# PeterFWS/Structure-PLP-SLAM

Measured on NVIDIA H100. Metric: frames_per_sec_extract_match_poseopt, higher is better.
Workload: dtype u8/f64

## Files before the change

### structure-plp-slam_b200/csrc/orb.cu

```cuda
#include "common.cuh"
#include <cuda.h>
#include <stdlib.h>
#include "brief_pattern.inc"
#include "quadtree_kernels.cuh"

namespace plp {

namespace {

constexpr int kMaxLevels = 16;
constexpr int kHalfPatch = 15;
constexpr int kCellSize = 64;
constexpr int kOverlap = 6;

struct LevelInfo {
    int w, h, pitch;
    size_t offset;
    size_t blur_offset;
    int cells_x, cells_y;
    int cell_base;
    int num_cells;
    int budget;
    int slot_base;
    int slot_cap;
    float scale_factor;
    float size;
};

struct CellDesc {
    short level, i, j, pad;
    short min_x, min_y, max_x, max_y;
};

struct BlurTile {
    short level, x0, y0, pad;
};

struct OrbDev {
    int num_levels, rows, cols;
    int num_cells;
    int total_slots;
    int out_cap;
    int ini_thr, min_thr;
    LevelInfo lv[kMaxLevels];
    int u_max[16];
    const uint8_t *img0;
    size_t img0_step, img0_frame_stride;
    const uint8_t *mask;
    size_t mask_step;
    uint8_t *pyr;
    size_t pyr_frame_bytes;
    uint8_t *blur;
    size_t blur_frame_bytes;
    const BlurTile *blur_tiles;
    int num_blur_tiles;
    const CellDesc *cells;
    uint32_t *cell_buf;
    int *cell_cnt;
    LevelKp *lvl_kp;
    int *lvl_cnt;
    uint8_t *qt_scratch;
    size_t qt_scratch_per_job;
    int *status;
};

__device__ __forceinline__ const uint8_t *level_ptr(const OrbDev &P, int b, int l) {
    return l == 0 ? P.img0 + (size_t)b * P.img0_frame_stride : P.pyr + (size_t)b * P.pyr_frame_bytes + P.lv[l].offset;
}
__device__ __forceinline__ int level_pitch(const OrbDev &P, int l) { return l == 0 ? (int)P.img0_step : P.lv[l].pitch; }

constexpr int kBtW = 64, kBtH = 32;
constexpr int kBoxW = 96, kBoxH = kBtH + 6, kBoxX = 16;
static_assert(kBoxW >= kBoxX + kBtW + 3 && kBoxW % 16 == 0 && kBoxX % 16 == 0 && kBtW % 16 == 0,
              "TMA box: 16-byte aligned start and extent covering the 3-pixel halo");
static_assert(kBoxH % 2 == 0 && kBtH % 2 == 0, "the blur passes work on pairs of rows");
constexpr int kBoxStage = (kBoxH * kBoxW + 127) & ~127;
constexpr int kTilePitch = kBoxW;
constexpr int kTileRows = kCellSize + kOverlap;

struct BlurMaps {
    CUtensorMap m[kMaxLevels];
};

__device__ __forceinline__ uint32_t smem_u32(const void *p) { return (uint32_t)__cvta_generic_to_shared(p); }

__device__ __forceinline__ void mbar_init(uint32_t bar) { asm volatile("mbarrier.init.shared::cta.b64 [%0], 1;" ::"r"(bar)); }

__device__ __forceinline__ bool mbar_wait(uint32_t bar, uint32_t parity) {
    uint32_t done = 0;
    for (int spin = 0; spin < (1 << 14) && !done; ++spin)
        asm volatile(
            "{\n\t.reg .pred p;\n\tmbarrier.try_wait.parity.shared::cta.b64 p, [%1], %2;\n\tselp.u32 %0, 1, 0, p;\n\t}"
            : "=r"(done)
            : "r"(bar), "r"(parity)
            : "memory");
    return done != 0;
}

__device__ __forceinline__ void mbar_expect_tx(uint32_t bar, uint32_t bytes) {
    asm volatile("mbarrier.arrive.expect_tx.shared::cta.b64 _, [%0], %1;" ::"r"(bar), "r"(bytes) : "memory");
}

__device__ __forceinline__ void tma_box_load(uint32_t dst, const CUtensorMap *tm, int x, int y, int f, uint32_t bar) {
    asm volatile(
        "cp.async.bulk.tensor.3d.shared::cluster.global.mbarrier::complete_tx::bytes [%0], [%1, {%2, %3, %4}], [%5];"
        ::"r"(dst), "l"(tm), "r"(x), "r"(y), "r"(f), "r"(bar)
        : "memory");
}

constexpr int kResizeRows = 8;
__global__ void __launch_bounds__(256) pyr_resize_kernel(OrbDev P, int l, const short4 *__restrict__ xtab,
                                                         const short4 *__restrict__ ytab) {
    const int b = blockIdx.y;
    const int dw = P.lv[l].w, dh = P.lv[l].h, dpitch = P.lv[l].pitch;
    const int quads = (dw + 3) >> 2, strips = (dh + kResizeRows - 1) / kResizeRows;
    const int q = blockIdx.x * blockDim.x + threadIdx.x;
    if (q >= quads * strips) return;
    const int strip = q / quads, x0 = (q - strip * quads) * 4;
    const uint8_t *src = level_ptr(P, b, l - 1);
    const int spitch = level_pitch(P, l - 1);
    uint8_t *dst = const_cast<uint8_t *>(level_ptr(P, b, l));
    int sx0[4], sx1[4], a0[4], a1[4];
#pragma unroll
    for (int k = 0; k < 4; ++k) {
        const short4 xt = xtab[min(x0 + k, dw - 1)];
        sx0[k] = xt.x;
        sx1[k] = xt.y;
        a0[k] = xt.z;
        a1[k] = xt.w;
    }
    const int y_end = min(dh, (strip + 1) * kResizeRows);
    for (int y = strip * kResizeRows; y < y_end; ++y) {
        const short4 yt = ytab[y];
        const uint8_t *S0 = src + (size_t)yt.x * spitch, *S1 = src + (size_t)yt.y * spitch;
        const int b0 = yt.z, b1 = yt.w;
        uint32_t packed = 0;
#pragma unroll
        for (int k = 0; k < 4; ++k) {
            const int r0 = S0[sx0[k]] * a0[k] + S0[sx1[k]] * a1[k];
            const int r1 = S1[sx0[k]] * a0[k] + S1[sx1[k]] * a1[k];
            const int v = (((b0 * (r0 >> 4)) >> 16) + ((b1 * (r1 >> 4)) >> 16) + 2) >> 2;
            packed |= (uint32_t)(v & 0xff) << (8 * k);
        }
        *reinterpret_cast<uint32_t *>(dst + (size_t)y * dpitch + x0) = packed;
    }
}

__device__ __forceinline__ uint32_t fast_m_pair(const uint8_t *pa, const uint8_t *pb) {
    const uint32_t v2 = ((uint32_t)pa[0] + 256u) | (((uint32_t)pb[0] + 256u) << 16);
    uint32_t d[16];
#define PLP_RING(k, off) d[k] = v2 - ((uint32_t)pa[off] | ((uint32_t)pb[off] << 16))
    PLP_RING(0, 3 * kTilePitch);
    PLP_RING(1, 3 * kTilePitch + 1);
    PLP_RING(2, 2 * kTilePitch + 2);
    PLP_RING(3, 1 * kTilePitch + 3);
    PLP_RING(4, 3);
    PLP_RING(5, -1 * kTilePitch + 3);
    PLP_RING(6, -2 * kTilePitch + 2);
    PLP_RING(7, -3 * kTilePitch + 1);
    PLP_RING(8, -3 * kTilePitch);
    PLP_RING(9, -3 * kTilePitch - 1);
    PLP_RING(10, -2 * kTilePitch - 2);
    PLP_RING(11, -1 * kTilePitch - 3);
    PLP_RING(12, -3);
    PLP_RING(13, 1 * kTilePitch - 3);
    PLP_RING(14, 2 * kTilePitch - 2);
    PLP_RING(15, 3 * kTilePitch - 1);
#undef PLP_RING
    uint32_t e[16], d2[16], e2[16], d4[16], e4[16];
#pragma unroll
    for (int k = 0; k < 16; ++k) e[k] = 0x02000200u - d[k];
#pragma unroll
    for (int k = 0; k < 16; ++k) {
        d2[k] = __vimin3_s16x2(d[k], d[(k + 1) & 15], d[(k + 1) & 15]);
        e2[k] = __vimin3_s16x2(e[k], e[(k + 1) & 15], e[(k + 1) & 15]);
    }
#pragma unroll
    for (int k = 0; k < 16; ++k) {
        d4[k] = __vimin3_s16x2(d2[k], d2[(k + 2) & 15], d2[(k + 2) & 15]);
        e4[k] = __vimin3_s16x2(e2[k], e2[(k + 2) & 15], e2[(k + 2) & 15]);
    }
    uint32_t best = 0u;
#pragma unroll
    for (int k = 0; k < 16; ++k) {
        const uint32_t d9 = __vimin3_s16x2(d4[k], d4[(k + 4) & 15], d[(k + 8) & 15]);
        const uint32_t e9 = __vimin3_s16x2(e4[k], e4[(k + 4) & 15], e[(k + 8) & 15]);
        best = __vimax3_s16x2(best, d9, e9);
    }
    return best;
}

__device__ __forceinline__ bool masked(const OrbDev &P, unsigned y, unsigned x, float scale) {
    return P.mask[(size_t)(int)(y * scale) * P.mask_step + (int)(x * scale)] == 0;
}


constexpr int kTileX = kPatchRadius % 16;
constexpr int kTestX = kTileX + 3;
static_assert(kCellSize % 16 == 0 && kTestX % 4 == 2, "the pretests below form their words for tested x = 2 (mod 4)");
static_assert(kTileX + kCellSize + kOverlap <= kTilePitch, "a cell row fits a tile row");
constexpr int kFastBox2Row = kTileRows - kBoxH;
static_assert(kFastBox2Row > 0 && kFastBox2Row <= kBoxH && (kFastBox2Row * kTilePitch) % 128 == 0,
              "two boxes cover the tile rows; the second lands 128-byte aligned");
constexpr int kFastStage = (kTileRows * kTilePitch + 127) & ~127;
constexpr int kCornerWords = 4;
static_assert(kCornerWords * 32 >= kTilePitch + 32, "corner bitmap row");

#define PLP_TW(y, k) T32[(y) * (kTilePitch / 4) + (k)]

__device__ __forceinline__ uint32_t compass4(const uint32_t *T32, int y, int k, uint32_t t4) {
    const uint32_t c = __funnelshift_r(PLP_TW(y, k), PLP_TW(y, k + 1), 16);
    const uint32_t up = __funnelshift_r(PLP_TW(y - 3, k), PLP_TW(y - 3, k + 1), 16);
    const uint32_t dn = __funnelshift_r(PLP_TW(y + 3, k), PLP_TW(y + 3, k + 1), 16);
    const uint32_t lf = __funnelshift_r(PLP_TW(y, k - 1), PLP_TW(y, k), 24);
    const uint32_t rt = __funnelshift_r(PLP_TW(y, k + 1), PLP_TW(y, k + 2), 8);
    const uint32_t a0 = __vcmpgtu4(__vabsdiffu4(c, dn), t4), a4 = __vcmpgtu4(__vabsdiffu4(c, rt), t4);
    const uint32_t a8 = __vcmpgtu4(__vabsdiffu4(c, up), t4), a12 = __vcmpgtu4(__vabsdiffu4(c, lf), t4);
    const uint32_t sv = (a4 | a12) & (a0 | a8);
    const uint32_t m = sv & 0x01010101u;
    return (m | (m >> 7) | (m >> 14) | (m >> 21)) & 0xfu;
}

__device__ __forceinline__ uint32_t even8_4(const uint32_t *T32, int y, int k, uint32_t k7) {
    const uint32_t c = __funnelshift_r(PLP_TW(y, k), PLP_TW(y, k + 1), 16);
    auto gt = [&](uint32_t ring) -> uint32_t {
        const uint32_t d = __vabsdiffu4(c, ring);
        return (((d & 0x7f7f7f7fu) + k7) | d) & 0x80808080u;
    };
    const uint32_t e0 = gt(__funnelshift_r(PLP_TW(y + 3, k), PLP_TW(y + 3, k + 1), 16));
    const uint32_t e2 = gt(PLP_TW(y + 2, k + 1));
// ... 554 lines not shown
                const uint32_t r[12] = {q0.x, q0.y, q0.z, q0.w, q1.x, q1.y, q1.z, q1.w, q2.x, q2.y, q2.z, q2.w};
                const int od = (cx - kHalfPatch) & 15, sh = 8 * (od & 3);
                switch (od >> 2) {
                    case 0: disc_row_sums<0>(r, sh, wu, wm, su, si); break;
                    case 1: disc_row_sums<1>(r, sh, wu, wm, su, si); break;
                    case 2: disc_row_sums<2>(r, sh, wu, wm, su, si); break;
                    default: disc_row_sums<3>(r, sh, wu, wm, su, si); break;
                }
            }
            int m10 = su, m01 = (lane - kHalfPatch) * si;
#pragma unroll
            for (int o = 16; o > 0; o >>= 1) {
                m10 += __shfl_xor_sync(0xffffffffu, m10, o);
                m01 += __shfl_xor_sync(0xffffffffu, m01, o);
            }
            const float angle = fast_atan2_deg((float)m01, (float)m10);

            const float ang_rad = (float)((double)angle * 3.14159265358979323846 / 180.0);
            const float ca = util_cos(ang_rad), sa = util_sin(ang_rad);
            const uint8_t *center = win + kWinHalf * kWinPitch + kWinHalf + ((cx - kWinHalf) & 15);
            int val = 0;
#pragma unroll
            for (int bit = 0; bit < 8; ++bit) {
                const int r1 = __float2int_rn(x1[bit] * sa + y1[bit] * ca), c1 = __float2int_rn(x1[bit] * ca - y1[bit] * sa);
                const int r2 = __float2int_rn(x2[bit] * sa + y2[bit] * ca), c2 = __float2int_rn(x2[bit] * ca - y2[bit] * sa);
                val |= (center[r1 * kWinPitch + c1] < center[r2 * kWinPitch + c2]) << bit;
            }
            desc_out[((size_t)b * P.out_cap + p0 + i) * 32 + lane] = (uint8_t)val;
            if (lane == i) my_angle = angle;
            __syncwarp();
        }
        if (lane < n) {
            plp_keypoint o;
            const float s = s_scale[ml];
            o.x = ml == 0 ? (float)mx : (float)mx * s;
            o.y = ml == 0 ? (float)my : (float)my * s;
            o.size = s_size[ml];
            o.angle = my_angle;
            o.response = (float)mresp;
            o.octave = ml;
            o.class_id = -1;
            kp_out[(size_t)b * P.out_cap + p0 + lane] = o;
        }
    }
}

}

}

using namespace plp;

constexpr auto kQtSmall = quadtree_kernel<kNodeCapSmall, kCandCapSmall, kQtThreadsSmall, kQtMinBlocksSmall>;
constexpr auto kQtLarge = quadtree_kernel<kNodeCap, kCandCapLarge, kQtThreadsLarge, kQtMinBlocksLarge>;
static_assert(kQtMaxLevels >= kMaxLevels, "the quadtree job holds every pyramid level");

static QtJob qt_job(const OrbDev &D) {
    QtJob J;
    J.num_levels = D.num_levels;
    J.num_cells = D.num_cells;
    J.total_slots = D.total_slots;
    for (int l = 0; l < D.num_levels; ++l) {
        const LevelInfo &V = D.lv[l];
        J.lv[l] = QtLevel{V.w, V.h, V.cell_base, V.num_cells, V.budget, V.slot_base, V.slot_cap};
    }
    J.cell_buf = D.cell_buf;
    J.cell_cnt = D.cell_cnt;
    J.lvl_kp = D.lvl_kp;
    J.lvl_cnt = D.lvl_cnt;
    J.scratch = D.qt_scratch;
    J.scratch_per_job = D.qt_scratch_per_job;
    J.status = D.status;
    return J;
}

struct plp_orb {
    plp_ctx *ctx = nullptr;
    plp_orb_params params;
    int rows = 0, cols = 0, max_batch = 0;
    OrbDev dev;
    std::vector<float> scale_factors, inv_scale_factors, level_sigma_sq, inv_level_sigma_sq;
    std::vector<uint32_t> num_keypts_per_level;
    std::vector<CellDesc> cells;
    short4 *d_xtab[kMaxLevels] = {nullptr};
    short4 *d_ytab[kMaxLevels] = {nullptr};
    CellDesc *d_cells = nullptr;
    uint8_t *d_pyr = nullptr;
    uint8_t *d_blur = nullptr;
    BlurTile *d_blur_tiles = nullptr;
    std::vector<BlurTile> blur_tiles;
    uint8_t *d_img = nullptr;
    uint8_t *d_mask = nullptr;
    uint32_t *d_cell_buf = nullptr;
    int *d_cell_cnt = nullptr;
    LevelKp *d_lvl_kp = nullptr;
    int *d_lvl_cnt = nullptr;
    uint8_t *d_qt_scratch = nullptr;
    int *d_status = nullptr;
    plp_keypoint *d_kp = nullptr;
    uint8_t *d_desc = nullptr;
    int32_t *d_n = nullptr;
    size_t qt_smem = 0;
    bool qt_small = false;
    BlurMaps maps;
    bool maps_ok = false;
    const uint8_t *map0_img = nullptr;
    size_t map0_step = 0;
    int map0_batch = 0;
    int last_batch = 0;
    const uint8_t *last_img0 = nullptr;
    size_t last_step = 0;
};

typedef CUresult (*EncodeTiledFn)(CUtensorMap *, CUtensorMapDataType, cuuint32_t, void *, const cuuint64_t *, const cuuint64_t *,
                                  const cuuint32_t *, const cuuint32_t *, CUtensorMapInterleave, CUtensorMapSwizzle,
                                  CUtensorMapL2promotion, CUtensorMapFloatOOBfill);
static EncodeTiledFn tensor_map_encoder() {
    static EncodeTiledFn fn = []() -> EncodeTiledFn {
        void *p = nullptr;
        cudaDriverEntryPointQueryResult q;
        if (cudaGetDriverEntryPoint("cuTensorMapEncodeTiled", &p, cudaEnableDefault, &q) != cudaSuccess ||
            q != cudaDriverEntryPointSuccess)
            return nullptr;
        return (EncodeTiledFn)p;
    }();
    return fn;
}
static bool encode_level_map(CUtensorMap *m, const uint8_t *base, int w, int h, int frames, size_t pitch, size_t frame_stride) {
    EncodeTiledFn enc = tensor_map_encoder();
    if (!enc || ((uintptr_t)base & 15) || (pitch & 15) || (frame_stride & 15) || w < 1 || h < 1 || frames < 1) return false;
    const cuuint64_t dims[3] = {(cuuint64_t)w, (cuuint64_t)h, (cuuint64_t)frames};
    const cuuint64_t strides[2] = {(cuuint64_t)pitch, (cuuint64_t)frame_stride};
    const cuuint32_t box[3] = {(cuuint32_t)kBoxW, (cuuint32_t)kBoxH, 1u}, estr[3] = {1u, 1u, 1u};
    return enc(m, CU_TENSOR_MAP_DATA_TYPE_UINT8, 3, (void *)base, dims, strides, box, estr, CU_TENSOR_MAP_INTERLEAVE_NONE,
               CU_TENSOR_MAP_SWIZZLE_NONE, CU_TENSOR_MAP_L2_PROMOTION_L2_128B, CU_TENSOR_MAP_FLOAT_OOB_FILL_NONE) == CUDA_SUCCESS;
}


static void build_resize_tables(int sw, int sh, int dw, int dh, std::vector<short4> &xt, std::vector<short4> &yt) {
    const double inv_scale_x = (double)dw / sw, inv_scale_y = (double)dh / sh;
    const double scale_x = 1. / inv_scale_x, scale_y = 1. / inv_scale_y;
    xt.resize(dw);
    yt.resize(dh);
    for (int dx = 0; dx < dw; ++dx) {
        float fx = (float)((dx + 0.5) * scale_x - 0.5);
        int sx = cv_floor(fx);
        fx -= sx;
        if (sx < 0) {
            fx = 0;
            sx = 0;
        }
        if (sx >= sw - 1) {
            fx = 0;
            sx = sw - 1;
        }
        short4 t;
        t.x = (short)sx;
        t.y = (short)std::min(sx + 1, sw - 1);
        t.z = (short)lrintf((1.f - fx) * 2048);
        t.w = (short)lrintf(fx * 2048);
        xt[dx] = t;
    }
    for (int dy = 0; dy < dh; ++dy) {
        float fy = (float)((dy + 0.5) * scale_y - 0.5);
        int sy = cv_floor(fy);
        fy -= sy;
        short4 t;
        t.x = (short)std::min(std::max(sy, 0), sh - 1);
        t.y = (short)std::min(std::max(sy + 1, 0), sh - 1);
        t.z = (short)lrintf((1.f - fy) * 2048);
        t.w = (short)lrintf(fy * 2048);
        yt[dy] = t;
    }
}

extern "C" {

void plp_orb_destroy(plp_orb *o) {
    if (!o) return;
    cudaSetDevice(o->ctx->device);
    cudaStreamSynchronize(o->ctx->stream);
    for (int l = 0; l < kMaxLevels; ++l) {
        if (o->d_xtab[l]) cudaFree(o->d_xtab[l]);
        if (o->d_ytab[l]) cudaFree(o->d_ytab[l]);
    }
    void *ptrs[] = {o->d_blur, o->d_blur_tiles, o->d_cells, o->d_pyr, o->d_img, o->d_mask, o->d_cell_buf, o->d_cell_cnt, o->d_lvl_kp,
                    o->d_lvl_cnt, o->d_qt_scratch, o->d_status, o->d_kp, o->d_desc, o->d_n};
    for (void *p : ptrs)
        if (p) cudaFree(p);
    delete o;
}

plp_status plp_orb_create(plp_ctx *ctx, const plp_orb_params *params, int rows, int cols, int max_batch,
                          plp_orb **out) {
    PLP_REQUIRE(ctx && params && out, "null pointer");
    *out = nullptr;
    PLP_REQUIRE(rows > 0 && cols > 0 && max_batch > 0, "image size / batch");
    PLP_REQUIRE(params->num_levels >= 1 && params->num_levels <= kMaxLevels, "num_levels in [1,16]");
    PLP_REQUIRE(params->scale_factor > 1.0f || params->num_levels == 1, "scale_factor > 1");
    PLP_REQUIRE(cols <= 2047 + 2 * kPatchRadius && rows <= 1023 + 2 * kPatchRadius,
                "image larger than 2085 x 1061 (packed candidate coordinates)");
    PLP_REQUIRE(params->ini_fast_thr < 255 && params->min_fast_thr >= 1 && params->min_fast_thr <= params->ini_fast_thr,
                "FAST thresholds: 1 <= min <= ini < 255");
    PLP_CUDA_TRY(cudaSetDevice(ctx->device));
    plp_orb *o = new plp_orb();
    o->ctx = ctx;
    o->params = *params;
    o->rows = rows;
    o->cols = cols;
    o->max_batch = max_batch;
    const unsigned L = params->num_levels;
    o->scale_factors.assign(L, 1.0f);
    o->inv_scale_factors.assign(L, 1.0f);
    o->level_sigma_sq.assign(L, 1.0f);
    o->inv_level_sigma_sq.assign(L, 1.0f);
    for (unsigned l = 1; l < L; ++l) o->scale_factors[l] = params->scale_factor * o->scale_factors[l - 1];
    for (unsigned l = 1; l < L; ++l) o->inv_scale_factors[l] = (1.0f / params->scale_factor) * o->inv_scale_factors[l - 1];
    {
        float s = 1.0f;
        for (unsigned l = 1; l < L; ++l) {
            s = params->scale_factor * s;
            o->level_sigma_sq[l] = s * s;
            o->inv_level_sigma_sq[l] = 1.0f / (s * s);
        }
    }
    o->num_keypts_per_level.resize(L);
    {
        double desired = params->max_num_keypts * (1.0 - 1.0 / params->scale_factor) /
                         (1.0 - std::pow(1.0 / params->scale_factor, static_cast<double>(L)));
        if (L == 1) desired = params->max_num_keypts;
        unsigned total = 0;
        for (unsigned l = 0; l + 1 < L; ++l) {
            o->num_keypts_per_level[l] = (unsigned)std::round(desired);
            total += o->num_keypts_per_level[l];
            desired *= 1.0 / params->scale_factor;
        }
        o->num_keypts_per_level[L - 1] = (unsigned)std::max((int)params->max_num_keypts - (int)total, 0);
    }
    OrbDev &D = o->dev;
    memset(&D, 0, sizeof(D));
    D.num_levels = (int)L;
    D.rows = rows;
    D.cols = cols;
    D.ini_thr = (int)params->ini_fast_thr;
    D.min_thr = (int)params->min_fast_thr;
    {
        const unsigned vmax = (unsigned)std::floor(kHalfPatch * std::sqrt(2.0) / 2 + 1);
        const unsigned vmin = (unsigned)std::ceil(kHalfPatch * std::sqrt(2.0) / 2);
        for (unsigned v = 0; v <= vmax; ++v)
            D.u_max[v] = (int)std::round(std::sqrt((double)kHalfPatch * kHalfPatch - (double)v * v));
        for (unsigned v = kHalfPatch, v0 = 0; vmin <= v; --v) {
            while (D.u_max[v0] == D.u_max[v0 + 1]) ++v0;
            D.u_max[v] = (int)v0;
            ++v0;
        }
    }
    int qt_max_slots = 0, qt_max_cells = 0;
    size_t pyr_bytes = 0, blur_bytes = 0;
    int slot_base = 0, cell_base = 0;
    plp_status st = PLP_OK;
    for (unsigned l = 0; l < L; ++l) {
        LevelInfo &V = D.lv[l];
        if (l == 0) {
            V.w = cols;
            V.h = rows;
        } else {
            const double scale = o->scale_factors[l];
            V.w = (int)std::round(cols * 1.0 / scale);
            V.h = (int)std::round(rows * 1.0 / scale);
// ... 5 lines not shown
        V.blur_offset = blur_bytes;
        blur_bytes += (size_t)V.pitch * V.h + 256;
        blur_bytes = (blur_bytes + 255) & ~(size_t)255;
        for (int y0 = 0; y0 < V.h; y0 += kBtH)
            for (int x0 = 0; x0 < V.w; x0 += kBtW) o->blur_tiles.push_back(BlurTile{(short)l, (short)x0, (short)y0, 0});
        V.budget = (int)o->num_keypts_per_level[l];
        V.scale_factor = o->scale_factors[l];
        V.size = (float)(unsigned)(31 * o->scale_factors[l]);
        V.slot_base = slot_base;
        {
            int g0 = 1;
            if (V.w > 2 * kPatchRadius && V.h > 2 * kPatchRadius) {
                const double ratio = (double)(V.w - 2 * kPatchRadius) / (V.h - 2 * kPatchRadius);
                g0 = ratio > 1 ? (int)std::round(ratio) : (int)std::round(1 / ratio);
            }
            V.slot_cap = 4 * std::max(V.budget, g0) + 8;
        }
        slot_base += V.slot_cap;
        V.cell_base = cell_base;
        V.num_cells = 0;
        qt_max_slots = std::max(qt_max_slots, V.slot_cap);
        if (V.slot_cap > kNodeCap) {
            set_error("orb: level %u budget %d exceeds the quadtree node capacity", l, V.budget);
            st = PLP_ERR_CAPACITY;
        }
        if (V.w > 2 * kPatchRadius && V.h > 2 * kPatchRadius && V.w >= 1 && V.h >= 1) {
            const unsigned min_bx = kPatchRadius, min_by = kPatchRadius;
            const unsigned max_bx = V.w - kPatchRadius, max_by = V.h - kPatchRadius;
            const unsigned width = max_bx - min_bx, height = max_by - min_by;
            const unsigned ncols = width / kCellSize + 1, nrows = height / kCellSize + 1;
            V.cells_x = (int)ncols;
            V.cells_y = (int)nrows;
            for (unsigned i = 0; i < nrows; ++i) {
                const unsigned min_y = min_by + i * kCellSize;
                if (max_by - kOverlap <= min_y || max_by < kOverlap) continue;
                unsigned max_y = min_y + kCellSize + kOverlap;
                if (max_by < max_y) max_y = max_by;
                for (unsigned j = 0; j < ncols; ++j) {
                    const unsigned min_x = min_bx + j * kCellSize;
                    if (max_bx - kOverlap <= min_x || max_bx < kOverlap) continue;
                    unsigned max_x = min_x + kCellSize + kOverlap;
                    if (max_bx < max_x) max_x = max_bx;
                    CellDesc c;
                    c.level = (short)l;
                    c.i = (short)i;
                    c.j = (short)j;
                    c.pad = 0;
                    c.min_x = (short)min_x;
                    c.min_y = (short)min_y;
                    c.max_x = (short)max_x;
                    c.max_y = (short)max_y;
                    o->cells.push_back(c);
                    V.num_cells++;
                }
            }
        }
        cell_base += V.num_cells;
        qt_max_cells = std::max(qt_max_cells, V.num_cells);
    }
    if (st == PLP_OK && qt_max_cells + 1 > 2 * (qt_max_slots <= kNodeCapSmall ? kNodeCapSmall : kNodeCap)) {
        set_error("orb: a pyramid level of %d FAST cells exceeds the quadtree's cell capacity", qt_max_cells);
        st = PLP_ERR_CAPACITY;
    }
    if (st != PLP_OK) {
        delete o;
        return st;
    }
    D.num_cells = cell_base;
    D.total_slots = slot_base;
    D.out_cap = slot_base;
    D.pyr_frame_bytes = pyr_bytes ? pyr_bytes : 256;
    D.blur_frame_bytes = blur_bytes ? blur_bytes : 256;
    D.num_blur_tiles = (int)o->blur_tiles.size();
    const size_t B = (size_t)max_batch;
#define ORB_ALLOC(ptr, bytes)                                              \
    do {                                                                   \
        cudaError_t e_ = cudaMalloc((void **)&(ptr), (bytes) ? (bytes) : 256); \
        if (e_ != cudaSuccess) {                                           \
            set_error("orb: cudaMalloc(%zu) failed: %s", (size_t)(bytes), cudaGetErrorString(e_)); \
            plp_orb_destroy(o);                                            \
            return PLP_ERR_CUDA;                                           \
        }                                                                  \
    } while (0)
    for (unsigned l = 1; l < L; ++l) {
        std::vector<short4> xt, yt;
        build_resize_tables(D.lv[l - 1].w, D.lv[l - 1].h, D.lv[l].w, D.lv[l].h, xt, yt);
        ORB_ALLOC(o->d_xtab[l], xt.size() * sizeof(short4));
        ORB_ALLOC(o->d_ytab[l], yt.size() * sizeof(short4));
        cudaMemcpy(o->d_xtab[l], xt.data(), xt.size() * sizeof(short4), cudaMemcpyHostToDevice);
        cudaMemcpy(o->d_ytab[l], yt.data(), yt.size() * sizeof(short4), cudaMemcpyHostToDevice);
    }
    ORB_ALLOC(o->d_cells, o->cells.size() * sizeof(CellDesc));
    if (!o->cells.empty())
        cudaMemcpy(o->d_cells, o->cells.data(), o->cells.size() * sizeof(CellDesc), cudaMemcpyHostToDevice);
    ORB_ALLOC(o->d_pyr, B * D.pyr_frame_bytes);
    ORB_ALLOC(o->d_blur, B * D.blur_frame_bytes);
    ORB_ALLOC(o->d_blur_tiles, o->blur_tiles.size() * sizeof(BlurTile));
    if (!o->blur_tiles.empty())
        cudaMemcpy(o->d_blur_tiles, o->blur_tiles.data(), o->blur_tiles.size() * sizeof(BlurTile), cudaMemcpyHostToDevice);
    ORB_ALLOC(o->d_img, B * (size_t)rows * cols);
    ORB_ALLOC(o->d_mask, (size_t)rows * cols);
    ORB_ALLOC(o->d_cell_buf, B * (size_t)D.num_cells * kCellCap * sizeof(uint32_t));
    ORB_ALLOC(o->d_cell_cnt, B * (size_t)D.num_cells * sizeof(int));
    ORB_ALLOC(o->d_lvl_kp, B * (size_t)D.total_slots * sizeof(LevelKp));
    ORB_ALLOC(o->d_lvl_cnt, B * L * sizeof(int));
    D.qt_scratch_per_job = qt_scratch_bytes_per_job();
    ORB_ALLOC(o->d_qt_scratch, B * L * D.qt_scratch_per_job);
    ORB_ALLOC(o->d_status, B * sizeof(int));
    ORB_ALLOC(o->d_kp, B * (size_t)D.out_cap * sizeof(plp_keypoint));
    ORB_ALLOC(o->d_desc, B * (size_t)D.out_cap * 32);
    ORB_ALLOC(o->d_n, B * sizeof(int32_t));
#undef ORB_ALLOC
    D.pyr = o->d_pyr;
    D.blur = o->d_blur;
    D.blur_tiles = o->d_blur_tiles;
    D.cells = o->d_cells;
    D.cell_buf = o->d_cell_buf;
    D.cell_cnt = o->d_cell_cnt;
    D.lvl_kp = o->d_lvl_kp;
    D.lvl_cnt = o->d_lvl_cnt;
    D.qt_scratch = o->d_qt_scratch;
    D.status = o->d_status;
    o->maps_ok = true;
    memset(&o->maps, 0, sizeof(o->maps));
    for (unsigned l = 1; l < L && o->maps_ok; ++l)
        o->maps_ok = encode_level_map(&o->maps.m[l], o->d_pyr + D.lv[l].offset, D.lv[l].w, D.lv[l].h, max_batch, D.lv[l].pitch,
                                      D.pyr_frame_bytes);
    o->qt_small = qt_max_slots <= kNodeCapSmall;
    plp_status so;
    if (o->qt_small) {
        o->qt_smem = qt_smem_bytes<kNodeCapSmall, kCandCapSmall, kQtThreadsSmall>();
        so = ensure_smem_optin((const void *)kQtSmall, o->qt_smem, "quadtree_kernel<small>");
    } else {
        o->qt_smem = qt_smem_bytes<kNodeCap, kCandCapLarge, kQtThreadsLarge>();
        so = ensure_smem_optin((const void *)kQtLarge, o->qt_smem, "quadtree_kernel<large>");
    }
    if (so != PLP_OK) {
        plp_orb_destroy(o);
        return so;
    }
    *out = o;
    return PLP_OK;
}

int plp_orb_capacity(const plp_orb *o) { return o ? o->dev.out_cap : 0; }

plp_status plp_orb_get_tables(const plp_orb *o, float *sf, float *isf, float *ls, float *ils, uint32_t *nk) {
    PLP_REQUIRE(o, "orb");
    for (int l = 0; l < o->dev.num_levels; ++l) {
        if (sf) sf[l] = o->scale_factors[l];
        if (isf) isf[l] = o->inv_scale_factors[l];
        if (ls) ls[l] = o->level_sigma_sq[l];
        if (ils) ils[l] = o->inv_level_sigma_sq[l];
        if (nk) nk[l] = o->num_keypts_per_level[l];
    }
    return PLP_OK;
}

static plp_status orb_run(plp_orb *o, const uint8_t *d_imgs, int batch, size_t step, const uint8_t *d_mask,
                          size_t mask_step, plp_keypoint *d_kp, uint8_t *d_desc, int32_t *d_n, int32_t *d_status) {
    plp_ctx *ctx = o->ctx;
    OrbDev D = o->dev;
    D.img0 = d_imgs;
    D.img0_step = step;
    D.img0_frame_stride = step * (size_t)o->rows;
    D.mask = d_mask;
    D.mask_step = mask_step;
    D.status = d_status ? d_status : o->d_status;
    o->last_batch = batch;
    o->last_img0 = d_imgs;
    o->last_step = step;
    PLP_CUDA_TRY(cudaMemsetAsync(D.status, 0, (size_t)batch * sizeof(int), ctx->stream));
    for (int l = 1; l < D.num_levels; ++l) {
        const int quads = ((D.lv[l].w + 3) >> 2) * ((D.lv[l].h + kResizeRows - 1) / kResizeRows);
        if (quads <= 0) continue;
        dim3 grid(div_up(quads, 256), batch);
        PLP_LAUNCH(ctx, pyr_resize_kernel, grid, 256, 0, D, l, o->d_xtab[l], o->d_ytab[l]);
    }
    bool tma = o->maps_ok;
    if (tma && (o->map0_img != d_imgs || o->map0_step != step || o->map0_batch != batch)) {
        tma = encode_level_map(&o->maps.m[0], d_imgs, D.lv[0].w, D.lv[0].h, batch, step, D.img0_frame_stride);
        o->map0_img = tma ? d_imgs : nullptr;
        o->map0_step = step;
        o->map0_batch = batch;
    }
    if (D.num_cells > 0) {
        dim3 grid(D.num_cells, batch), grid_run(div_up(D.num_cells, kFastRun), batch);
        if (tma)
            PLP_LAUNCH(ctx, fast_cells_tma_kernel, grid_run, 256, 0, o->maps, D, kFastRun);
        else
            PLP_LAUNCH(ctx, fast_cells_kernel_v2, grid, 256, 0, D);
    }
    if (D.num_blur_tiles > 0) {
        dim3 grid(D.num_blur_tiles, batch), grid_run(div_up(D.num_blur_tiles, kBlurRun), batch);
        if (tma)
            PLP_LAUNCH(ctx, blur_tiles_tma_kernel, grid_run, kBlurThreads, 0, o->maps, D, kBlurRun);
        else
            PLP_LAUNCH(ctx, blur_tiles_kernel, grid, kBlurThreads, 0, D);
    }
    {
        dim3 grid(D.num_levels, batch);
        if (ctx->timing) plp::timing_begin(ctx, o->qt_small ? "quadtree_kernel<1024>" : "quadtree_kernel<2048>");
        const QtJob J = qt_job(D);
        if (o->qt_small)
            kQtSmall<<<grid, kQtThreadsSmall, o->qt_smem, ctx->stream>>>(J);
        else
            kQtLarge<<<grid, kQtThreadsLarge, o->qt_smem, ctx->stream>>>(J);
        if (ctx->timing) plp::timing_end(ctx);
        ctx->launches++;
    }
    {
        const int kp_est = std::max(256, (int)o->params.max_num_keypts);
        dim3 grid(div_up(std::min(D.total_slots, kp_est), kDescWarps * kDescRun), batch);
        PLP_LAUNCH(ctx, describe_kernel, grid, kDescWarps * 32, 0, D, d_kp, d_desc, d_n);
    }
    PLP_CHECK_LAUNCH();
    return PLP_OK;
}

plp_status plp_orb_extract_batch_dev(plp_orb *o, const uint8_t *d_imgs, int batch, size_t step, plp_keypoint *d_kp,
                                     uint8_t *d_desc, int32_t *d_n, int32_t *d_status) {
    PLP_REQUIRE(o && d_imgs && d_kp && d_desc && d_n, "null pointer");
    PLP_REQUIRE(batch >= 1 && batch <= o->max_batch, "batch exceeds the handle's max_batch");
    PLP_REQUIRE(step >= (size_t)o->cols, "step < cols");
    PLP_CUDA_TRY(cudaSetDevice(o->ctx->device));
    return orb_run(o, d_imgs, batch, step, nullptr, 0, d_kp, d_desc, d_n, d_status);
}

static plp_status orb_extract_host(plp_orb *o, const uint8_t *imgs, int batch, size_t step, const uint8_t *mask,
                                   size_t mask_step, plp_keypoint *kp_out, uint8_t *desc_out, int32_t *n_out) {
    plp_ctx *ctx = o->ctx;
    PLP_CUDA_TRY(cudaSetDevice(ctx->device));
    const size_t rows = o->rows, cols = o->cols;
    PLP_CUDA_TRY(cudaMemcpy2DAsync(o->d_img, cols, imgs, step, cols, rows * (size_t)batch, cudaMemcpyHostToDevice,
                                   ctx->stream));
    const uint8_t *d_mask = nullptr;
    if (mask) {
        PLP_CUDA_TRY(cudaMemcpy2DAsync(o->d_mask, cols, mask, mask_step, cols, rows, cudaMemcpyHostToDevice, ctx->stream));
        d_mask = o->d_mask;
    }
    PLP_TRY(orb_run(o, o->d_img, batch, cols, d_mask, cols, o->d_kp, o->d_desc, o->d_n, nullptr));
    const size_t cap = o->dev.out_cap;
    PLP_CUDA_TRY(cudaMemcpyAsync(n_out, o->d_n, (size_t)batch * 4, cudaMemcpyDeviceToHost, ctx->stream));
    PLP_CUDA_TRY(cudaMemcpyAsync(kp_out, o->d_kp, (size_t)batch * cap * sizeof(plp_keypoint), cudaMemcpyDeviceToHost,
                                 ctx->stream));
    PLP_CUDA_TRY(cudaMemcpyAsync(desc_out, o->d_desc, (size_t)batch * cap * 32, cudaMemcpyDeviceToHost, ctx->stream));
    std::vector<int> status(batch);
    PLP_CUDA_TRY(cudaMemcpyAsync(status.data(), o->d_status, (size_t)batch * 4, cudaMemcpyDeviceToHost, ctx->stream));
    PLP_CUDA_TRY(cudaStreamSynchronize(ctx->stream));
    for (int b = 0; b < batch; ++b)
        if (status[b] != 0) {
            set_error("orb: capacity overflow in frame %d (code %d)", b, status[b]);
            return PLP_ERR_CAPACITY;
        }
    return PLP_OK;
}

plp_status plp_orb_extract(plp_orb *o, const uint8_t *img, int rows, int cols, size_t step, const uint8_t *mask,
                           size_t mask_step, plp_keypoint *kp_out, uint8_t *desc_out, int *n_out) {
    PLP_REQUIRE(o && n_out, "null pointer");
// ... 85 lines not shown
```

Baseline: 89590.

## Fuse pyramid resize levels into tiled shared-memory kernel with host-built plan

Replaces the one-launch-per-level bilinear resize with a fused pyramid kernel. Each block loads the source region for its tile into shared memory with cp.async, then computes several successive levels in ping-pong shared buffers and writes each level's owned region to global memory. A host-side planner picks tile shapes and groups levels into launches that fit a shared-memory budget. When the taps allow it, a byte_perm/dp2a word path replaces per-byte loads. This removes per-level launches and global round trips between levels, but adds halo recomputation, more host planning, and higher shared-memory use.

Result: faster. 90810, median of 6 (+1.4%).

```diff
diff --git a/structure-plp-slam_b200/csrc/orb.cu b/structure-plp-slam_b200/csrc/orb.cu
--- a/structure-plp-slam_b200/csrc/orb.cu
+++ b/structure-plp-slam_b200/csrc/orb.cu
@@ -2,6 +2,7 @@
 #include <cuda.h>
 #include <stdlib.h>
 #include "brief_pattern.inc"
+#include "pyramid_kernels.cuh"
 #include "quadtree_kernels.cuh"
 
 namespace plp {
@@ -9,6 +10,7 @@
 namespace {
 
 constexpr int kMaxLevels = 16;
+static_assert(kMaxLevels == kPyrMaxLevels, "the pyramid plan covers every level");
 constexpr int kHalfPatch = 15;
 constexpr int kCellSize = 64;
 constexpr int kOverlap = 6;
@@ -108,44 +110,6 @@
         : "memory");
 }
 
-constexpr int kResizeRows = 8;
-__global__ void __launch_bounds__(256) pyr_resize_kernel(OrbDev P, int l, const short4 *__restrict__ xtab,
-                                                         const short4 *__restrict__ ytab) {
-    const int b = blockIdx.y;
-    const int dw = P.lv[l].w, dh = P.lv[l].h, dpitch = P.lv[l].pitch;
-    const int quads = (dw + 3) >> 2, strips = (dh + kResizeRows - 1) / kResizeRows;
-    const int q = blockIdx.x * blockDim.x + threadIdx.x;
-    if (q >= quads * strips) return;
-    const int strip = q / quads, x0 = (q - strip * quads) * 4;
-    const uint8_t *src = level_ptr(P, b, l - 1);
-    const int spitch = level_pitch(P, l - 1);
-    uint8_t *dst = const_cast<uint8_t *>(level_ptr(P, b, l));
-    int sx0[4], sx1[4], a0[4], a1[4];
-#pragma unroll
-    for (int k = 0; k < 4; ++k) {
-        const short4 xt = xtab[min(x0 + k, dw - 1)];
-        sx0[k] = xt.x;
-        sx1[k] = xt.y;
-        a0[k] = xt.z;
-        a1[k] = xt.w;
-    }
-    const int y_end = min(dh, (strip + 1) * kResizeRows);
-    for (int y = strip * kResizeRows; y < y_end; ++y) {
-        const short4 yt = ytab[y];
-        const uint8_t *S0 = src + (size_t)yt.x * spitch, *S1 = src + (size_t)yt.y * spitch;
-        const int b0 = yt.z, b1 = yt.w;
-        uint32_t packed = 0;
-#pragma unroll
-        for (int k = 0; k < 4; ++k) {
-            const int r0 = S0[sx0[k]] * a0[k] + S0[sx1[k]] * a1[k];
-            const int r1 = S1[sx0[k]] * a0[k] + S1[sx1[k]] * a1[k];
-            const int v = (((b0 * (r0 >> 4)) >> 16) + ((b1 * (r1 >> 4)) >> 16) + 2) >> 2;
-            packed |= (uint32_t)(v & 0xff) << (8 * k);
-        }
-        *reinterpret_cast<uint32_t *>(dst + (size_t)y * dpitch + x0) = packed;
-    }
-}
-
 __device__ __forceinline__ uint32_t fast_m_pair(const uint8_t *pa, const uint8_t *pb) {
     const uint32_t v2 = ((uint32_t)pa[0] + 256u) | (((uint32_t)pb[0] + 256u) << 16);
     uint32_t d[16];
@@ -866,8 +830,8 @@
     std::vector<float> scale_factors, inv_scale_factors, level_sigma_sq, inv_level_sigma_sq;
     std::vector<uint32_t> num_keypts_per_level;
     std::vector<CellDesc> cells;
-    short4 *d_xtab[kMaxLevels] = {nullptr};
-    short4 *d_ytab[kMaxLevels] = {nullptr};
+    PyrPlan pyr_plan;
+    uint8_t *d_pyr_plan = nullptr;
     CellDesc *d_cells = nullptr;
     uint8_t *d_pyr = nullptr;
     uint8_t *d_blur = nullptr;
@@ -921,54 +885,13 @@
 }
 
 
-static void build_resize_tables(int sw, int sh, int dw, int dh, std::vector<short4> &xt, std::vector<short4> &yt) {
-    const double inv_scale_x = (double)dw / sw, inv_scale_y = (double)dh / sh;
-    const double scale_x = 1. / inv_scale_x, scale_y = 1. / inv_scale_y;
-    xt.resize(dw);
-    yt.resize(dh);
-    for (int dx = 0; dx < dw; ++dx) {
-        float fx = (float)((dx + 0.5) * scale_x - 0.5);
-        int sx = cv_floor(fx);
-        fx -= sx;
-        if (sx < 0) {
-            fx = 0;
-            sx = 0;
-        }
-        if (sx >= sw - 1) {
-            fx = 0;
-            sx = sw - 1;
-        }
-        short4 t;
-        t.x = (short)sx;
-        t.y = (short)std::min(sx + 1, sw - 1);
-        t.z = (short)lrintf((1.f - fx) * 2048);
-        t.w = (short)lrintf(fx * 2048);
-        xt[dx] = t;
-    }
-    for (int dy = 0; dy < dh; ++dy) {
-        float fy = (float)((dy + 0.5) * scale_y - 0.5);
-        int sy = cv_floor(fy);
-        fy -= sy;
-        short4 t;
-        t.x = (short)std::min(std::max(sy, 0), sh - 1);
-        t.y = (short)std::min(std::max(sy + 1, 0), sh - 1);
-        t.z = (short)lrintf((1.f - fy) * 2048);
-        t.w = (short)lrintf(fy * 2048);
-        yt[dy] = t;
-    }
-}
-
 extern "C" {
 
 void plp_orb_destroy(plp_orb *o) {
     if (!o) return;
     cudaSetDevice(o->ctx->device);
     cudaStreamSynchronize(o->ctx->stream);
-    for (int l = 0; l < kMaxLevels; ++l) {
-        if (o->d_xtab[l]) cudaFree(o->d_xtab[l]);
-        if (o->d_ytab[l]) cudaFree(o->d_ytab[l]);
-    }
-    void *ptrs[] = {o->d_blur, o->d_blur_tiles, o->d_cells, o->d_pyr, o->d_img, o->d_mask, o->d_cell_buf, o->d_cell_cnt, o->d_lvl_kp,
+    void *ptrs[] = {o->d_pyr_plan, o->d_blur, o->d_blur_tiles, o->d_cells, o->d_pyr, o->d_img, o->d_mask, o->d_cell_buf, o->d_cell_cnt, o->d_lvl_kp,
                     o->d_lvl_cnt, o->d_qt_scratch, o->d_status, o->d_kp, o->d_desc, o->d_n};
     for (void *p : ptrs)
         if (p) cudaFree(p);
@@ -1140,14 +1063,21 @@
             return PLP_ERR_CUDA;                                           \
         }                                                                  \
     } while (0)
-    for (unsigned l = 1; l < L; ++l) {
-        std::vector<short4> xt, yt;
-        build_resize_tables(D.lv[l - 1].w, D.lv[l - 1].h, D.lv[l].w, D.lv[l].h, xt, yt);
-        ORB_ALLOC(o->d_xtab[l], xt.size() * sizeof(short4));
-        ORB_ALLOC(o->d_ytab[l], yt.size() * sizeof(short4));
-        cudaMemcpy(o->d_xtab[l], xt.data(), xt.size() * sizeof(short4), cudaMemcpyHostToDevice);
-        cudaMemcpy(o->d_ytab[l], yt.data(), yt.size() * sizeof(short4), cudaMemcpyHostToDevice);
-    }
+    {
+        int w[kMaxLevels], h[kMaxLevels];
+        for (unsigned l = 0; l < L; ++l) {
+            w[l] = D.lv[l].w;
+            h[l] = D.lv[l].h;
+        }
+        if (!pyr_make_plan(w, h, (int)L, kPyrSmemBudget, kPyrBands, &o->pyr_plan)) {
+            set_error("orb: no pyramid plan fits %zu bytes of shared memory at %d x %d", kPyrSmemBudget, cols, rows);
+            plp_orb_destroy(o);
+            return PLP_ERR_CAPACITY;
+        }
+    }
+    ORB_ALLOC(o->d_pyr_plan, o->pyr_plan.blob.size());
+    if (!o->pyr_plan.blob.empty())
+        cudaMemcpy(o->d_pyr_plan, o->pyr_plan.blob.data(), o->pyr_plan.blob.size(), cudaMemcpyHostToDevice);
     ORB_ALLOC(o->d_cells, o->cells.size() * sizeof(CellDesc));
     if (!o->cells.empty())
         cudaMemcpy(o->d_cells, o->cells.data(), o->cells.size() * sizeof(CellDesc), cudaMemcpyHostToDevice);
@@ -1185,7 +1115,11 @@
         o->maps_ok = encode_level_map(&o->maps.m[l], o->d_pyr + D.lv[l].offset, D.lv[l].w, D.lv[l].h, max_batch, D.lv[l].pitch,
                                       D.pyr_frame_bytes);
     o->qt_small = qt_max_slots <= kNodeCapSmall;
-    plp_status so;
+    plp_status so = ensure_smem_optin((const void *)pyramid_kernel, o->pyr_plan.max_smem, "pyramid_kernel");
+    if (so != PLP_OK) {
+        plp_orb_destroy(o);
+        return so;
+    }
     if (o->qt_small) {
         o->qt_smem = qt_smem_bytes<kNodeCapSmall, kCandCapSmall, kQtThreadsSmall>();
         so = ensure_smem_optin((const void *)kQtSmall, o->qt_smem, "quadtree_kernel<small>");
@@ -1229,11 +1163,18 @@
     o->last_img0 = d_imgs;
     o->last_step = step;
     PLP_CUDA_TRY(cudaMemsetAsync(D.status, 0, (size_t)batch * sizeof(int), ctx->stream));
-    for (int l = 1; l < D.num_levels; ++l) {
-        const int quads = ((D.lv[l].w + 3) >> 2) * ((D.lv[l].h + kResizeRows - 1) / kResizeRows);
-        if (quads <= 0) continue;
-        dim3 grid(div_up(quads, 256), batch);
-        PLP_LAUNCH(ctx, pyr_resize_kernel, grid, 256, 0, D, l, o->d_xtab[l], o->d_ytab[l]);
+    {
+        int pitch[kPyrMaxLevels] = {0};
+        size_t offset[kPyrMaxLevels] = {0};
+        for (int l = 0; l < D.num_levels; ++l) {
+            pitch[l] = D.lv[l].pitch;
+            offset[l] = D.lv[l].offset;
+        }
+        for (const PyrLaunch &Lh : o->pyr_plan.launches) {
+            const PyrJob J = pyr_job(o->pyr_plan, Lh, o->d_pyr_plan, pitch, offset, d_imgs, step, D.img0_frame_stride, D.pyr,
+                                     D.pyr_frame_bytes);
+            PLP_LAUNCH(ctx, pyramid_kernel, dim3(Lh.num_tiles, batch), kPyrThreads, Lh.smem, J);
+        }
     }
     bool tma = o->maps_ok;
     if (tma && (o->map0_img != d_imgs || o->map0_step != step || o->map0_batch != batch)) {
diff --git a/structure-plp-slam_b200/csrc/pyramid_kernels.cuh b/structure-plp-slam_b200/csrc/pyramid_kernels.cuh
--- /dev/null
+++ b/structure-plp-slam_b200/csrc/pyramid_kernels.cuh
@@ -0,0 +1,373 @@
+#pragma once
+#include <math.h>
+#include <stddef.h>
+#include <stdint.h>
+#include <string.h>
+
+#include <algorithm>
+#include <vector>
+
+#include "devmath.cuh"
+
+namespace plp {
+
+constexpr int kPyrMaxLevels = 16;
+constexpr int kPyrThreads = 256;
+constexpr int kPyrRowGroup = 8;
+constexpr int kPyrBands = 12;
+constexpr size_t kPyrSmemBudget = 56 * 1024;
+constexpr int kPyrMinBlocks = 4;
+
+struct PyrSpan {
+    int16_t y0, y1, x0, x1;
+};
+struct PyrTileLevel {
+    PyrSpan need, own;
+};
+
+__host__ __device__ inline bool pyr_empty(const PyrSpan &s) { return s.y1 <= s.y0 || s.x1 <= s.x0; }
+__host__ __device__ inline int pyr_base(const PyrSpan &s) { return s.x0 & ~15; }
+__host__ __device__ inline int pyr_stride(const PyrSpan &s) { return ((s.x1 + 15) & ~15) - (s.x0 & ~15); }
+inline size_t pyr_span_bytes(const PyrSpan &s) { return pyr_empty(s) ? 0 : (size_t)(s.y1 - s.y0) * pyr_stride(s) + 16; }
+
+
+inline void pyr_resize_tables(int sw, int sh, int dw, int dh, std::vector<short4> &xt, std::vector<short4> &yt) {
+    const double inv_scale_x = (double)dw / sw, inv_scale_y = (double)dh / sh;
+    const double scale_x = 1. / inv_scale_x, scale_y = 1. / inv_scale_y;
+    xt.resize(dw);
+    yt.resize(dh);
+    for (int dx = 0; dx < dw; ++dx) {
+        float fx = (float)((dx + 0.5) * scale_x - 0.5);
+        int sx = cv_floor(fx);
+        fx -= sx;
+        if (sx < 0) {
+            fx = 0;
+            sx = 0;
+        }
+        if (sx >= sw - 1) {
+            fx = 0;
+            sx = sw - 1;
+        }
+        short4 t;
+        t.x = (short)sx;
+        t.y = (short)std::min(sx + 1, sw - 1);
+        t.z = (short)lrintf((1.f - fx) * 2048);
+        t.w = (short)lrintf(fx * 2048);
+        xt[dx] = t;
+    }
+    for (int dy = 0; dy < dh; ++dy) {
+        float fy = (float)((dy + 0.5) * scale_y - 0.5);
+        int sy = cv_floor(fy);
+        fy -= sy;
+        short4 t;
+        t.x = (short)std::min(std::max(sy, 0), sh - 1);
+        t.y = (short)std::min(std::max(sy + 1, 0), sh - 1);
+        t.z = (short)lrintf((1.f - fy) * 2048);
+        t.w = (short)lrintf(fy * 2048);
+        yt[dy] = t;
+    }
+}
+
+struct PyrLaunch {
+    int first, last;
+    int num_tiles;
+    size_t tiles_off;
+    size_t buf_b;
+    size_t smem;
+};
+
+struct PyrPlan {
+    std::vector<PyrLaunch> launches;
+    std::vector<uint8_t> blob;
+    size_t xoff[kPyrMaxLevels] = {}, yoff[kPyrMaxLevels] = {};
+    uint32_t word_taps = 0;
+    size_t max_smem = 0;
+};
+
+namespace pyr_detail {
+
+inline PyrSpan hull(const PyrSpan &a, const PyrSpan &b) {
+    if (pyr_empty(a)) return b;
+    if (pyr_empty(b)) return a;
+    return PyrSpan{std::min(a.y0, b.y0), std::max(a.y1, b.y1), std::min(a.x0, b.x0), std::max(a.x1, b.x1)};
+}
+
+inline PyrSpan own_span(int w, int h, int k, int K, int j, int X) {
+    auto xb = [&](int i) { return i == 0 ? 0 : i == X ? w : (int)((int64_t)i * w / X) & ~15; };
+    return PyrSpan{(int16_t)(((int64_t)k * h + K - 1) / K), (int16_t)(((int64_t)(k + 1) * h + K - 1) / K), (int16_t)xb(j),
+                   (int16_t)xb(j + 1)};
+}
+
+inline bool tiles_for(const int *w, const int *h, const std::vector<short4> *xt, const std::vector<short4> *yt, int a, int e,
+                      int K, int X, size_t budget, std::vector<PyrTileLevel> &out, size_t *buf_b, size_t *smem) {
+    const int n = e - a + 1;
+    out.assign((size_t)K * X * n, PyrTileLevel{});
+    size_t max_a = 0, max_b = 0;
+    for (int k = 0; k < K; ++k)
+        for (int j = 0; j < X; ++j) {
+            PyrTileLevel *T = out.data() + ((size_t)k * X + j) * n;
+            for (int l = e; l > a; --l) {
+                const PyrSpan own = own_span(w[l], h[l], k, K, j, X);
+                if (!pyr_empty(own)) T[l - a].own = own;
+                const PyrSpan nd = hull(T[l - a].need, T[l - a].own);
+                T[l - a].need = nd;
+                if (pyr_empty(nd)) continue;
+                const PyrSpan src{yt[l][nd.y0].x, (int16_t)(yt[l][nd.y1 - 1].y + 1), xt[l][nd.x0].x, (int16_t)(xt[l][nd.x1 - 1].y + 1)};
+                T[l - 1 - a].need = hull(T[l - 1 - a].need, src);
+            }
+            for (int i = 0; i < n; ++i) {
+                size_t &m = (i & 1) ? max_b : max_a;
+                m = std::max(m, pyr_span_bytes(T[i].need));
+            }
+        }
+    *buf_b = (max_a + 15) & ~(size_t)15;
+    *smem = *buf_b + max_b;
+    return *smem <= budget;
+}
+
+}
+
+inline bool pyr_make_plan(const int *w, const int *h, int L, size_t budget, int bands, PyrPlan *P) {
+    using namespace pyr_detail;
+    *P = PyrPlan{};
+    std::vector<short4> xt[kPyrMaxLevels], yt[kPyrMaxLevels];
+    int top = 0;
+    for (int l = 1; l < L && w[l] > 0 && h[l] > 0; ++l) {
+        pyr_resize_tables(w[l - 1], h[l - 1], w[l], h[l], xt[l], yt[l]);
+        top = l;
+        bool ok = true;
+        for (int q = 0; 4 * q < w[l]; ++q)
+            ok = ok && xt[l][std::min(4 * q + 3, w[l] - 1)].y - 4 * (xt[l][4 * q].x >> 2) <= 11;
+        if (ok) P->word_taps |= 1u << l;
+    }
+    std::vector<PyrTileLevel> tiles;
+    bands = std::max(1, bands);
+    for (int a = 0; a < top;) {
+        size_t buf_b = 0, smem = 0;
+        const int kmax = std::max(bands, (h[a] + 15) / 16), xmax = std::max(1, (w[a] + 63) / 64);
+        auto fits = [&](int e) {
+            for (int X = 1;; X = std::min(2 * X, xmax)) {
+                for (int K = bands; K <= kmax; K += std::max(1, K / 4))
+                    if (tiles_for(w, h, xt, yt, a, e, K, X, budget, tiles, &buf_b, &smem)) return true;
+                if (X == xmax) return false;
+            }
+        };
+        int e = top;
+        while (e > a && !fits(e)) --e;
+        if (e == a) return false;
+        PyrLaunch Lh;
+        Lh.first = a;
+        Lh.last = e;
+        Lh.num_tiles = (int)(tiles.size() / (size_t)(e - a + 1));
+        Lh.tiles_off = P->blob.size();
+        Lh.buf_b = buf_b;
+        Lh.smem = smem;
+        P->blob.resize(P->blob.size() + tiles.size() * sizeof(PyrTileLevel));
+        memcpy(P->blob.data() + Lh.tiles_off, tiles.data(), tiles.size() * sizeof(PyrTileLevel));
+        P->launches.push_back(Lh);
+        P->max_smem = std::max(P->max_smem, smem);
+        a = e;
+    }
+    for (int l = 1; l <= top; ++l) {
+        P->xoff[l] = P->blob.size();
+        P->yoff[l] = P->xoff[l] + xt[l].size() * sizeof(short4);
+        P->blob.resize(P->yoff[l] + yt[l].size() * sizeof(short4));
+        memcpy(P->blob.data() + P->xoff[l], xt[l].data(), xt[l].size() * sizeof(short4));
+        memcpy(P->blob.data() + P->yoff[l], yt[l].data(), yt[l].size() * sizeof(short4));
+    }
+    return true;
+}
+
+
+struct PyrJob {
+    int first, last;
+    const PyrTileLevel *tiles;
+    int buf_b;
+    uint32_t word_taps;
+    const short4 *xtab[kPyrMaxLevels], *ytab[kPyrMaxLevels];
+    int pitch[kPyrMaxLevels];
+    size_t offset[kPyrMaxLevels];
+    const uint8_t *src;
+    size_t src_step, src_frame;
+    int src_vec;
+    uint8_t *pyr;
+    size_t pyr_frame;
+};
+
+inline PyrJob pyr_job(const PyrPlan &P, const PyrLaunch &Lh, const uint8_t *blob, const int *pitch, const size_t *offset,
+                      const uint8_t *img0, size_t step0, size_t frame0, uint8_t *pyr, size_t pyr_frame) {
+    PyrJob J;
+    memset(&J, 0, sizeof(J));
+    J.first = Lh.first;
+    J.last = Lh.last;
+    J.tiles = reinterpret_cast<const PyrTileLevel *>(blob + Lh.tiles_off);
+    J.buf_b = (int)Lh.buf_b;
+    J.word_taps = P.word_taps;
+    for (int l = Lh.first + 1; l <= Lh.last; ++l) {
+        J.xtab[l] = reinterpret_cast<const short4 *>(blob + P.xoff[l]);
+        J.ytab[l] = reinterpret_cast<const short4 *>(blob + P.yoff[l]);
+    }
+    for (int l = 0; l < kPyrMaxLevels; ++l) {
+        J.pitch[l] = pitch[l];
+        J.offset[l] = offset[l];
+    }
+    if (Lh.first == 0) {
+        J.src = img0;
+        J.src_step = step0;
+        J.src_frame = frame0;
+    } else {
+        J.src = pyr + offset[Lh.first];
+        J.src_step = (size_t)pitch[Lh.first];
+        J.src_frame = pyr_frame;
+    }
+    J.src_vec = (((uintptr_t)J.src | J.src_step | J.src_frame) & 15) == 0;
+    J.pyr = pyr;
+    J.pyr_frame = pyr_frame;
+    return J;
+}
+
+namespace {
+
+__device__ __forceinline__ void pyr_cp16(uint8_t *dst, const uint8_t *src) {
+#ifdef PLP_CTA_EMU
+    memcpy(dst, src, 16);
+#else
+    asm volatile("cp.async.cg.shared.global [%0], [%1], 16;" ::"r"((uint32_t)__cvta_generic_to_shared(dst)), "l"(src)
+                 : "memory");
+#endif
+}
+__device__ __forceinline__ void pyr_cp_wait() {
+#ifndef PLP_CTA_EMU
+    asm volatile("cp.async.wait_all;" ::: "memory");
+#endif
+}
+
+__device__ __forceinline__ uint32_t pyr_vert(uint32_t B0, uint32_t h0, uint32_t B1, uint32_t h1) {
+    return (__umulhi(B0, h0) + __umulhi(B1, h1) + 2) >> 2;
+}
+
+__device__ __forceinline__ void pyr_level(const uint8_t *sb, const PyrSpan S, uint8_t *db, const PyrSpan D,
+                                          const short4 *__restrict__ xtab, const short4 *__restrict__ ytab, bool words) {
+    const int sbase = pyr_base(S), sstride = pyr_stride(S);
+    const int dbase = pyr_base(D), dstride = pyr_stride(D);
+    const int quads = dstride >> 2, groups = (D.y1 - D.y0 + kPyrRowGroup - 1) / kPyrRowGroup;
+    for (int it = (int)threadIdx.x; it < quads * groups; it += kPyrThreads) {
+        const int g = it / quads, q = it - g * quads;
+        const int x = dbase + 4 * q;
+        int s0[4], s1[4];
+        uint32_t wt[4];
+#pragma unroll
+        for (int k = 0; k < 4; ++k) {
+            const short4 xt = __ldg(xtab + min(max(x + k, (int)D.x0), (int)D.x1 - 1));
+            s0[k] = xt.x - sbase;
+            s1[k] = xt.y - sbase;
+            wt[k] = (uint32_t)(uint16_t)xt.z | (uint32_t)(uint16_t)xt.w << 16;
+        }
+        const int y_beg = D.y0 + g * kPyrRowGroup, y_end = min((int)D.y1, y_beg + kPyrRowGroup);
+        uint8_t *out = db + (size_t)(y_beg - D.y0) * dstride + 4 * q;
+        if (words) {
+            const int w0 = s0[0] >> 2;
+            uint32_t sel_lo[2], sel_hi[2];
+#pragma unroll
+            for (int p = 0; p < 2; ++p) {
+                const int o[4] = {s0[2 * p] - 4 * w0, s1[2 * p] - 4 * w0, s0[2 * p + 1] - 4 * w0, s1[2 * p + 1] - 4 * w0};
+                sel_lo[p] = sel_hi[p] = 0;
+#pragma unroll
+                for (int j = 0; j < 4; ++j) {
+                    sel_lo[p] |= (uint32_t)(o[j] < 8 ? o[j] : 0) << (4 * j);
+                    sel_hi[p] |= (uint32_t)(o[j] < 8 ? j : o[j] - 4) << (4 * j);
+                }
+            }
+            auto hpass = [&](int sy, uint32_t *hh) {
+                const uint32_t *r = reinterpret_cast<const uint32_t *>(sb + (size_t)sy * sstride) + w0;
+                const uint32_t u0 = r[0], u1 = r[1], u2 = r[2];
+#pragma unroll
+                for (int p = 0; p < 2; ++p) {
+                    const uint32_t T = __byte_perm(__byte_perm(u0, u1, sel_lo[p]), u2, sel_hi[p]);
+                    hh[2 * p] = __dp2a_lo(wt[2 * p], T, 0u) >> 4;
+                    hh[2 * p + 1] = __dp2a_hi(wt[2 * p + 1], T, 0u) >> 4;
+                }
+            };
+            short4 yts[kPyrRowGroup];
+#pragma unroll
+            for (int r = 0; r < kPyrRowGroup; ++r) yts[r] = __ldg(ytab + min(y_beg + r, (int)D.y1 - 1));
+#pragma unroll
+            for (int r = 0; r < kPyrRowGroup; ++r) {
+                const short4 yt = yts[r];
+                uint32_t h0[4], h1[4];
+                hpass(yt.x - S.y0, h0);
+                hpass(yt.y - S.y0, h1);
+                const uint32_t B0 = (uint32_t)(uint16_t)yt.z << 16, B1 = (uint32_t)(uint16_t)yt.w << 16;
+                const uint32_t v01 = __byte_perm(pyr_vert(B0, h0[0], B1, h1[0]), pyr_vert(B0, h0[1], B1, h1[1]), 0x0040);
+                const uint32_t v23 = __byte_perm(pyr_vert(B0, h0[2], B1, h1[2]), pyr_vert(B0, h0[3], B1, h1[3]), 0x0040);
+                if (y_beg + r < y_end) *reinterpret_cast<uint32_t *>(out + (size_t)r * dstride) = __byte_perm(v01, v23, 0x5410);
+            }
+        } else {
+            for (int y = y_beg; y < y_end; ++y) {
+                const short4 yt = __ldg(ytab + y);
+                const uint8_t *R0 = sb + (size_t)(yt.x - S.y0) * sstride, *R1 = sb + (size_t)(yt.y - S.y0) * sstride;
+                const uint32_t B0 = (uint32_t)(uint16_t)yt.z << 16, B1 = (uint32_t)(uint16_t)yt.w << 16;
+                uint32_t word = 0;
+#pragma unroll
+                for (int k = 0; k < 4; ++k) {
+                    const uint32_t a0 = wt[k] & 0xffffu, a1 = wt[k] >> 16;
+                    const uint32_t r0 = R0[s0[k]] * a0 + R0[s1[k]] * a1, r1 = R1[s0[k]] * a0 + R1[s1[k]] * a1;
+                    word |= pyr_vert(B0, r0 >> 4, B1, r1 >> 4) << (8 * k);
+                }
+                *reinterpret_cast<uint32_t *>(out) = word;
+                out += dstride;
+            }
+        }
+    }
+}
+
+__global__ void __launch_bounds__(kPyrThreads, kPyrMinBlocks) pyramid_kernel(PyrJob J) {
+    PLP_DYNAMIC_SMEM(smem);
+    const int t = (int)threadIdx.x, b = (int)blockIdx.y, n = J.last - J.first + 1;
+    const PyrTileLevel *T = J.tiles + (size_t)blockIdx.x * n;
+    {
+        const PyrSpan s = T[0].need;
+        if (!pyr_empty(s)) {
+            const int base = pyr_base(s), stride = pyr_stride(s), rows = s.y1 - s.y0;
+            const uint8_t *src = J.src + (size_t)b * J.src_frame + (size_t)s.y0 * J.src_step;
+            if (J.src_vec) {
+                const int chunks = stride >> 4;
+                for (int i = t; i < rows * chunks; i += kPyrThreads) {
+                    const int r = i / chunks, c = i - r * chunks;
+                    pyr_cp16(smem + (size_t)r * stride + 16 * c, src + (size_t)r * J.src_step + base + 16 * c);
+                }
+                pyr_cp_wait();
+            } else {
+                const int w = s.x1 - s.x0;
+                for (int i = t; i < rows * w; i += kPyrThreads) {
+                    const int r = i / w, c = i - r * w;
+                    smem[(size_t)r * stride + s.x0 - base + c] = src[(size_t)r * J.src_step + s.x0 + c];
+                }
+            }
+        }
+        __syncthreads();
+    }
+    for (int i = 1; i < n; ++i) {
+        const int l = J.first + i;
+        const uint8_t *sb = smem + ((i - 1) & 1 ? J.buf_b : 0);
+        uint8_t *db = smem + (i & 1 ? J.buf_b : 0);
+        const PyrSpan D = T[i].need, O = T[i].own;
+        if (!pyr_empty(D)) pyr_level(sb, T[i - 1].need, db, D, J.xtab[l], J.ytab[l], (J.word_taps >> l) & 1u);
+        __syncthreads();
+        if (!pyr_empty(O)) {
+            const int dbase = pyr_base(D), dstride = pyr_stride(D), pitch = J.pitch[l];
+            const int chunks = (((O.x1 + 15) & ~15) - O.x0) >> 4, rows = O.y1 - O.y0;
+            uint8_t *dst = J.pyr + (size_t)b * J.pyr_frame + J.offset[l] + (size_t)O.y0 * pitch + O.x0;
+            const uint8_t *sp = db + (size_t)(O.y0 - D.y0) * dstride + (O.x0 - dbase);
+            for (int k = t; k < rows * chunks; k += kPyrThreads) {
+                const int r = k / chunks, c = k - r * chunks;
+                *reinterpret_cast<uint4 *>(dst + (size_t)r * pitch + 16 * c) =
+                    *reinterpret_cast<const uint4 *>(sp + (size_t)r * dstride + 16 * c);
+            }
+        }
+    }
+}
+
+}
+
+}
```
